# ehsan5890/optical-rl-gym-qot-aware

Hardware: AMD Instinct MI355X
Metric: env steps/sec (whole node) + blocking-prob parity, NSFNET RMSA 320 slots (higher is better)
Workload: dtype u64 bitmap + f64 statistics

## Files before the change

### optical-rl-gym-qot-aware_amd/csrc/orlg_api.hip

```cpp
#include "orlg_host.h"
#include "orlg_group_plan.h"
#include "orlg_wave.h"

struct orlg_env : OrlgHandle {
    OrlgParams p = {};
    int resident_blocks = 0;
    int group_mode = 0;
    OrlgGroupLayout group[3] = {};
    int group_usage_resident[ORLG_GROUP_WAVES + 1] = {};
    int group_resident[3][ORLG_GROUP_WAVES + 1] = {};
    uint4 *llog = nullptr;
    uint32_t *progress = nullptr;
    int allow_rejection = 0;
    std::vector<uint8_t> path_se;
    double *gn_table = nullptr;
    bool gn_protect = false;
    double *audit_table = nullptr;
};
enum { X_ACTIONS, X_GSNR, X_CAUSE, X_CAUSE_COUNTS, X_MARGIN };
static_assert(X_MARGIN < ORLG_EXTRA_SLOTS, "OrlgHandle::extra");

#define SYNC_CHECK(e) do { int rc_ = orlg_handle_sync_check(e); if (rc_) return rc_; } while (0)

__global__ void orlg_clear_state_kernel(OrlgParams p, int W, int keep_rng) {
    const size_t tid = (size_t)blockIdx.x * blockDim.x + threadIdx.x, nth = (size_t)gridDim.x * blockDim.x;
    for (size_t i = tid; i < (size_t)p.B * p.NW; i += nth) p.occ[i] = valid_mask(p.S, (int)(i % W));
    for (size_t i = tid; i < (size_t)p.B * p.Q; i += nth) {
        p.qtime[i] = __longlong_as_double((long long)ORLG_INF_BITS);
        p.qdesc[i] = 0;
    }
    for (size_t i = tid; i < (size_t)p.B * 4 * p.NBR; i += nth) p.hist[i] = 0;
    for (size_t i = tid; i < (size_t)p.B * 4 * p.E; i += nth) p.lstat[i] = 0.0;
    for (size_t i = tid; i < (size_t)p.B * p.lint_stride; i += nth) p.lint[i] = 0;
    for (size_t i = tid; i < (size_t)p.B; i += nth) {
        OrlgEnvScalars s;
        memset(&s, 0, sizeof(s));
        s.mt_idx = keep_rng ? p.scal[i].mt_idx : ORLG_MT_N;
        s.ring_pos = keep_rng ? p.scal[i].ring_pos : 0;
        s.ring_cnt = keep_rng ? p.scal[i].ring_cnt : 0;
        if (p.tr_arrival) { s.mt_idx = 0; s.ring_pos = 0; s.ring_cnt = 0; }
        p.scal[i] = s;
    }
}

__global__ __launch_bounds__(256) void orlg_simple_matrix_obs_kernel(const OrlgParams p, int W, uint8_t *out) {
    const size_t dim = (size_t)2 * p.N + (size_t)p.E * p.S;
    const size_t total = dim * p.B;
    for (size_t i = (size_t)blockIdx.x * blockDim.x + threadIdx.x; i < total; i += (size_t)gridDim.x * blockDim.x) {
        const size_t b = i / dim, q = i - b * dim;
        uint8_t v;
        if (q < (size_t)2 * p.N) {
            const OrlgEnvScalars *sc = p.scal + b;
            const int mn = sc->req_src < sc->req_dst ? sc->req_src : sc->req_dst;
            const int mx = sc->req_src < sc->req_dst ? sc->req_dst : sc->req_src;
            v = ((int)q == mn || (int)q == p.N + mx) ? 1 : 0;
        } else {
            const size_t r = q - 2 * p.N;
            const int link = (int)(r / p.S), s = (int)(r - (size_t)link * p.S);
            v = (uint8_t)((p.occ[b * p.NW + (size_t)link * W + (s >> 6)] >> (s & 63)) & 1ull);
        }
        out[i] = v;
    }
}

enum { EX_REQUEST, EX_COUNTERS, EX_TIME, EX_GRAPH, EX_RUNNING, EX_EPISODES, EX_HIST, EX_LSTAT };
__global__ void orlg_extract_kernel(OrlgParams p, int what, unsigned char *out) {
    const size_t tid = (size_t)blockIdx.x * blockDim.x + threadIdx.x, nth = (size_t)gridDim.x * blockDim.x;
    const size_t B = p.B;
    if (what == EX_REQUEST) {
        orlg_request *o = reinterpret_cast<orlg_request *>(out);
        for (size_t i = tid; i < B; i += nth) {
            const OrlgEnvScalars &s = p.scal[i];
            o[i].service_id = s.req_sid; o[i].src = s.req_src; o[i].dst = s.req_dst;
            o[i].bit_rate = reinterpret_cast<const int32_t *>(p.tables + p.t_bitrates)[s.req_br];
            o[i].arrival_time = s.req_arrival; o[i].holding_time = s.req_holding;
        }
    } else if (what == EX_COUNTERS) {
        int64_t *o = reinterpret_cast<int64_t *>(out);
        for (size_t i = tid; i < B * 8; i += nth) o[i] = p.scal[i / 8].c[i % 8];
    } else if (what == EX_TIME) {
        double *o = reinterpret_cast<double *>(out);
        for (size_t i = tid; i < B; i += nth) o[i] = p.scal[i].current_time;
    } else if (what == EX_GRAPH) {
        double *o = reinterpret_cast<double *>(out);
        for (size_t i = tid; i < B; i += nth) {
// ... 172 lines not shown


int orlg_create(const orlg_topology *t, const orlg_rmsa_config *c, int32_t batch, const uint64_t *seeds,
                uint64_t base_seed, int32_t device, orlg_env **out) {
    return orlg_create_traffic(t, c, batch, seeds, base_seed, device, nullptr, out);
}

static int rmsa_create(const orlg_topology *t, const orlg_rmsa_config *c, int32_t batch, const uint64_t *seeds, uint64_t base_seed,
                       int32_t device, const orlg_traffic *traffic, const orlg_trace *trace, orlg_env **out);
int orlg_create_traffic(const orlg_topology *t, const orlg_rmsa_config *c, int32_t batch, const uint64_t *seeds,
                        uint64_t base_seed, int32_t device, const orlg_traffic *traffic, orlg_env **out) {
    return rmsa_create(t, c, batch, seeds, base_seed, device, traffic, nullptr, out);
}
int orlg_create_trace(const orlg_topology *t, const orlg_rmsa_config *c, int32_t batch, int32_t device, const orlg_trace *trace,
                      orlg_env **out) {
    if (!trace) return fail(ORLG_ERR_INVALID, "null argument");
    return rmsa_create(t, c, batch, nullptr, 0, device, nullptr, trace, out);
}
int64_t orlg_trace_length(orlg_env *e) { return e ? e->trace.length : ORLG_ERR_INVALID; }
int64_t orlg_trace_position(orlg_env *e) { return e ? e->trace.position : ORLG_ERR_INVALID; }

static int rmsa_create(const orlg_topology *t, const orlg_rmsa_config *c, int32_t batch, const uint64_t *seeds, uint64_t base_seed,
                       int32_t device, const orlg_traffic *traffic, const orlg_trace *trace, orlg_env **out) {
    if (!t || !c || !out) return fail(ORLG_ERR_INVALID, "null argument");
    *out = nullptr;
    const int N = t->num_nodes, E = t->num_links, K = t->k_paths, S = c->num_slots, NBR = c->num_bit_rates;
    if (batch < 1) return fail(ORLG_ERR_INVALID, "batch must be >= 1");
    if (N < 2 || N > 64) return fail(ORLG_ERR_INVALID, "num_nodes %d not in 2..64", N);
    if (E < 1 || E > 255) return fail(ORLG_ERR_INVALID, "num_links %d not in 1..255", E);
    if (S < 1 || S > 512) return fail(ORLG_ERR_INVALID, "num_slots %d not in 1..512", S);
    const bool cont = c->bit_rate_cum == nullptr;
    if (NBR < 1 || NBR > (cont ? 256 : 64)) return fail(ORLG_ERR_INVALID, "num_bit_rates %d not in 1..%d", NBR, cont ? 256 : 64);
    if (cont) {
        if (!c->bit_rates) return fail(ORLG_ERR_INVALID, "null argument");
        for (int b = 1; b < NBR; b++)
            if (c->bit_rates[b] != c->bit_rates[0] + b) return fail(ORLG_ERR_INVALID, "continuous bit rates must be lower .. higher, one apart");
    }
    if (t->num_paths < 1 || t->num_paths >= (1 << 14)) return fail(ORLG_ERR_INVALID, "num_paths %d not in 1..16383", t->num_paths);
    int W = (S + 63) / 64;
    if (W == 7) W = 8;
    if (K < 1 || K * W > 64) return fail(ORLG_ERR_INVALID, "k_paths * words_per_link = %d exceeds one wavefront", K * W);
    if (c->j < 1 || c->j > 16) return fail(ORLG_ERR_INVALID, "j %d not in 1..16", c->j);
    if ((!traffic && !trace && (!(c->arrival_lambda > 0) || !(c->holding_lambda > 0))) || !(c->channel_width > 0))
        return fail(ORLG_ERR_INVALID, "arrival_lambda, holding_lambda and channel_width must be positive");
    auto e = std::make_unique<orlg_env>();
    double arrival_lambda = c->arrival_lambda, holding_lambda = c->holding_lambda;
    int rc = orlg_traffic_check(&e->traffic, traffic, batch, &arrival_lambda, &holding_lambda);
    if (rc) return rc;
    if (c->stats_level < 0 || c->stats_level > 2) return fail(ORLG_ERR_INVALID, "bad stats_level");
    for (int i = 0; i < N * N; i++) {
        int s = i / N, d = i % N;
        if (s != d && (t->pair_path_count[i] != K || t->pair_path_base[i] < 0 || t->pair_path_base[i] + K > t->num_paths))
            return fail(ORLG_ERR_INVALID, "pair (%d,%d) does not have k=%d path records", s, d, K);
    }
    const OrlgTraceState &trace_state = e->trace;
    if (trace) {
        if (!c->bit_rates) return fail(ORLG_ERR_INVALID, "null argument");
        rc = orlg_trace_check(&e->trace, &e->traffic, trace, batch, N, NBR, c->bit_rates, cont, &arrival_lambda, &holding_lambda);
        if (rc) return rc;
    }
    rc = orlg_handle_open(e.get(), device);
    if (rc) return rc;
    e->W = W; e->num_paths = t->num_paths;
    OrlgParams &p = e->p;
    p.err_flag = e->err.dev;
    p.B = batch; p.N = N; p.E = E; p.S = S; p.K = K; p.NBR = NBR; p.NW = E * W;
    p.episode_length = c->episode_length; p.reward_mode = c->reward_mode; p.stats_level = c->stats_level; p.j = c->j;
    p.obs_dim = 1 + 2 * N + (2 * c->j + 3) * K;
    p.arrival_lambda = arrival_lambda; p.holding_lambda = holding_lambda;
    int Q = c->queue_capacity;
    if (Q <= 0 && trace) {
        const int by_trace = trace_state.peak + 1, by_spectrum = E * S / 2 + 1;
        Q = by_trace < by_spectrum ? by_trace : by_spectrum;
        if (Q > 4096)
            return fail(ORLG_ERR_INVALID, "trace: up to %d services run at once (the trace's peak %d, the spectrum's bound %d): more than the 4096 "
                                          "release-queue slots the LDS holds", Q - 1, trace_state.peak, by_spectrum - 1);
    } else if (Q <= 0) {
        double load = arrival_lambda / holding_lambda;
        Q = (int)(load + 10.0 * std::sqrt(load));
    }
    Q = ((Q + 15) / 16) * 16;
    if (Q < 64) Q = 64;
    if (Q > 4096) return fail(ORLG_ERR_INVALID, "queue_capacity %d too large for LDS (max 4096)", Q);
    p.Q = Q;
    {
        char msg[192];
        snprintf(msg, sizeof(msg), "a release queue overflowed (capacity %d): the service stays provisioned and is never "
                                   "released -- raise queue_capacity", Q);
        e->overflow_message = msg;
    }

    auto up16 = [](int v) { return (v + 15) & ~15; };
    int off = 0;
    p.l_occ = off; off = up16(off + p.NW * 8);
    p.l_qtime = off; off = up16(off + Q * 8);
    p.l_qdesc = off; off = up16(off + Q * 4);
    p.l_mt = off; off = up16(off + ORLG_MT_N * 4);
    p.l_lstat = off; off = up16(off + 4 * E * 8);
    p.l_hist = off; off = up16(off + 4 * NBR * 4);
    p.lint_stride = (E + 3) & ~3;
    p.l_lint = off; off = up16(off + p.lint_stride * 4);
    p.l_scratch = off; off = up16(off + (int)sizeof(OrlgEnvScalars));
    p.l_wsc = off; off = up16(off + (int)sizeof(OrlgWaveScalars));
    p.l_ring = off; off = up16(off + ORLG_RING * (8 + 8 + 4));
    p.l_wave_bytes = off;

    {
        OrlgBlob blob;
        p.t_pair = blob.put(t->pair_path_base, (size_t)N * N * 4);
        std::vector<OrlgPathRec> recs;
        rc = orlg_path_records(t, E, "path %d: link %d out of range", &recs);
        if (rc) return rc;
        for (int g = 0; g < t->num_paths; g++)
            if (t->path_se[g] < 1 || t->path_se[g] >= ORLG_NSLOT_STRIDE)
                return fail(ORLG_ERR_INVALID, "path %d: spectral efficiency %d not in 1..7", g, t->path_se[g]);
        p.t_recs = blob.put(recs.data(), recs.size() * sizeof(OrlgPathRec));
        e->path_se.assign(t->path_se, t->path_se + t->num_paths);
        std::vector<uint16_t> ns((size_t)NBR * ORLG_NSLOT_STRIDE, 0);
        for (int b = 0; b < NBR; b++)
            for (int se = 1; se < ORLG_NSLOT_STRIDE; se++) {
                double q = (double)c->bit_rates[b] / ((double)se * c->channel_width);
                double n = std::ceil(q) + 1;
                ns[(size_t)b * ORLG_NSLOT_STRIDE + se] = (uint16_t)(n > 65535 ? 65535 : n);
            }
        p.t_nslots = blob.put(ns.data(), ns.size() * 2);
        p.t_bitrates = blob.put(c->bit_rates, (size_t)NBR * 4);
        {
            std::vector<double> zc((size_t)NBR, 0.0);
            p.t_brcum = blob.put(cont ? zc.data() : c->bit_rate_cum, (size_t)NBR * 8);
        }
        p.br_width = cont ? NBR : 0;
        p.t_srccum = blob.put(c->src_cum, (size_t)N * 8);
        p.t_dstcum = blob.put(c->dst_cum, (size_t)N * N * 8);
        if (c->stats_level >= ORLG_STATS_FULL) {
            std::vector<double> divs(S + 1), inv(S / 2 + 2);
            for (int k = 0; k <= S; k++) divs[k] = (double)k / (double)S;
            inv[0] = 0.0;
            for (size_t k = 1; k < inv.size(); k++) inv[k] = 1.0 / (double)k;
            p.t_divs = blob.put(divs.data(), divs.size() * 8);
            p.t_inv = blob.put(inv.data(), inv.size() * 8);
        }
        p.tab_bytes = (int32_t)blob.bytes.size();
        p.l_outs = p.tab_bytes;
        p.l_shared_bytes = p.tab_bytes + up16(ORLG_NUM_OUTS * 8);
        unsigned char *d_blob;
        rc = orlg_handle_upload(e.get(), &d_blob, blob.bytes.data(), blob.bytes.size());
        if (rc) return rc;
        p.tables = d_blob;
    }
    {
        const size_t lds_cu = ORLG_LDS_BYTES;
        int wpb = 0, best_waves = 0;
        const int wave_cap = 16;
        for (int cand = ORLG_MAX_WAVES_PER_BLOCK; cand >= 1; cand >>= 1) {
            size_t blk = (size_t)p.l_shared_bytes + (size_t)cand * p.l_wave_bytes;
            if (blk > lds_cu) continue;
            int waves = (int)(lds_cu / blk) * cand;
            if (waves > wave_cap) waves = wave_cap;
            if (waves > best_waves) { best_waves = waves; wpb = cand; }
        }
        if (wpb == 0) {
            size_t need = (size_t)p.l_shared_bytes + (size_t)p.l_wave_bytes;
            return fail(ORLG_ERR_INVALID, "tables + one environment (%zu B) exceed the 160 KiB LDS", need);
        }
        e->waves_per_block = wpb;
        e->lds_block_bytes = (size_t)p.l_shared_bytes + (size_t)wpb * p.l_wave_bytes;
// ... 943 lines not shown
```

### optical-rl-gym-qot-aware_amd/csrc/orlg_group_body.h

```cpp
    static_assert(!DEFER || (STATS >= 2 && !HBMQ), "the deferred link statistics belong to long launches with full statistics");
    static_assert(!(TRACE && TRAFFIC), "a trace handle has no arrival rates");
    static_assert(!LEAN || DEFER, "the lean body belongs to the long launches");
    static_assert(!CAUSE || (!HBMQ && !DEFER), "the blocking cause belongs to the plain kind");
    static_assert(!ASSIGN || (!HBMQ && !DEFER), "the assignment rules belong to the plain kind");
    static_assert(!CUT || ASSIGN, "the fewest-cuts window is an assignment rule");
    static_assert(!USAGE || (ASSIGN && !CUT), "most-used windows and the best-window route are assignment rules of their own");
    extern __shared__ __align__(16) unsigned char smem[];
    stage_tables(smem, p);
    const int lane = threadIdx.x & 63;
    const int wib = uni((int)(threadIdx.x >> 6));
    const int g = lane >> 4, gl = lane & 15;
    const Tab tb = make_tab(smem, p);
    uint32_t *mt_lds = reinterpret_cast<uint32_t *>(smem + p.l_shared_bytes);
    int *mt_lock = reinterpret_cast<int *>(smem + p.l_shared_bytes + p.g_mt);
    if (threadIdx.x == 0) *mt_lock = 0;
    __syncthreads();
    unsigned char *wbase = smem + p.l_shared_bytes + p.g_mt + 16 + (size_t)wib * p.g_wave_bytes;
    u64 *occ = reinterpret_cast<u64 *>(wbase + p.g_occ) + g * p.NW;
    double *qtime = nullptr;
    uint32_t *qdesc = nullptr;
    if constexpr (!HBMQ) {
        qtime = reinterpret_cast<double *>(wbase + p.g_qtime) + g * p.Q;
        qdesc = reinterpret_cast<uint32_t *>(wbase + p.g_qdesc) + g * p.Q;
    }
    double *lst = DEFER ? nullptr : reinterpret_cast<double *>(wbase + p.g_lstat) + g * 4 * p.E;
    int32_t *lint = reinterpret_cast<int32_t *>(wbase + p.g_lint) + g * p.lint_stride;
    u64 *lsum = DEFER ? reinterpret_cast<u64 *>(wbase + p.g_lstat) + g * p.E : nullptr;

    const int E = p.E, S = p.S, K = p.K, N = p.N, NBR = p.NBR, Q = p.Q, NW = p.NW;
    constexpr bool NET = STATS >= 1;
    constexpr bool FULL = STATS >= 2;
    const double INF = __longlong_as_double((long long)ORLG_INF_BITS);
    const bool out_comp = !LEAN && (p.out_mask & ((1 << ORLG_OUT_COMPACT) | (1 << ORLG_OUT_COMPACT_DIFF))) != 0;
    SEC_DECL_G

    const int n_quads = (p.B + ORLG_GE - 1) / ORLG_GE;
    const int n_chunks = p.n_chunks > 1 ? p.n_chunks : 1;
    const int n_tix = n_quads * n_chunks;
    const int n_waves = (int)(gridDim.x * (blockDim.x >> 6));
    const int n_static = n_chunks > 1 ? 0 : (n_waves < n_tix ? n_waves : n_tix);
    int tix = (int)(blockIdx.x * (blockDim.x >> 6)) + wib;
    if (n_chunks == 1 && tix >= n_tix) return;
    uint32_t nxt_tk = 0;
    if (n_chunks > 1 && lane == 0) nxt_tk = atomicAdd(p.ticket, 1u);
    for (bool first = n_chunks == 1;; first = false) {
    if (!first) {
        if (p.ticket_stride) {
            tix += n_waves;
            if (tix >= n_tix) break;
        } else {
            const uint32_t tk = (uint32_t)__builtin_amdgcn_readfirstlane((int)nxt_tk) - p.ticket_base;
            if (tk >= (uint32_t)(n_tix - n_static)) break;
            tix = n_static + (int)tk;
        }
    }
    int chunk = 0, quad = tix;
    if (n_chunks > 1) { chunk = tix / n_quads; quad = tix - chunk * n_quads; }
    const int t0 = n_chunks > 1 ? chunk * p.chunk_steps : 0;
    SEC(1);
    if (!p.ticket_stride && lane == 0) nxt_tk = atomicAdd(p.ticket, 1u);
    if (chunk > 0) {
        if (lane == 0)
            while (__hip_atomic_load(p.progress + quad, __ATOMIC_RELAXED, __HIP_MEMORY_SCOPE_AGENT) < (uint32_t)chunk) __builtin_amdgcn_s_sleep(16);
        __builtin_amdgcn_fence(__ATOMIC_ACQUIRE, "agent");
        asm volatile("s_waitcnt vmcnt(0)" ::: "memory");
    }
    const int env_raw = quad * ORLG_GE + g;
    const bool act = env_raw < p.B;
    const int env = act ? env_raw : p.B - 1;

    const int env0 = quad * ORLG_GE;
    const int nact = p.B - env0 < ORLG_GE ? p.B - env0 : ORLG_GE;
    quad_copy(wbase + p.g_occ, p.occ + (size_t)env0 * NW, nact * NW * 8, lane);
    if (FULL && !DEFER) quad_copy(wbase + p.g_lstat, p.lstat + (size_t)env0 * 4 * E, nact * 4 * E * 8, lane);
    int32_t *ghist = p.hist + (size_t)env * 4 * NBR;
    if (NET) quad_copy(wbase + p.g_lint, p.lint + (size_t)env0 * p.lint_stride, nact * p.lint_stride * 4, lane);
    if (nact < ORLG_GE) {
        wave_sync();
        if (!act) {
            const int gs_ = nact - 1;
            for (int i = gl; i < NW; i += ORLG_GL) occ[i] = (reinterpret_cast<u64 *>(wbase + p.g_occ) + gs_ * NW)[i];
            if (FULL && !DEFER) for (int i = gl; i < 4 * E; i += ORLG_GL) lst[i] = (reinterpret_cast<double *>(wbase + p.g_lstat) + gs_ * 4 * E)[i];
            if (NET) for (int i = gl; i < p.lint_stride; i += ORLG_GL) lint[i] = (reinterpret_cast<int32_t *>(wbase + p.g_lint) + gs_ * p.lint_stride)[i];
        }
    }
    uint4 *llog = DEFER ? p.llog + (size_t)env * E * ORLG_LLOG_CAP : nullptr;
    if (DEFER) lst = p.lstat + (size_t)env * 4 * E;
    bool need_replay = false;
    const OrlgEnvScalars *gs = p.scal + env;
    double current_time = gs->current_time, req_arrival = gs->req_arrival, req_holding = gs->req_holding;
    double g_thr = gs->g_throughput, g_comp = gs->g_compactness, g_lu = gs->g_last_update;
    long long cnt = gs->c[gl & 7];
    long long sum_bitrate_running = gs->sum_bitrate_running, episodes_done = gs->episodes_done;
    int sum_sh = gs->sum_slots_hops, n_running = gs->n_running;
    int req_src = gs->req_src, req_dst = gs->req_dst, req_br = gs->req_br, req_sid = gs->req_sid;
    int mt_idx = gs->mt_idx, new_service = gs->new_service, q_overflow = gs->q_overflow;
    int ring_pos = gs->ring_pos, ring_cnt = gs->ring_cnt;
    int sum_span = gs->sum_span, sum_gaps = gs->sum_gaps;
    int eproc = (int)gs->c[2];
    wave_sync();
    double comp_cur = 1.0;
    if (NET) comp_cur = network_compactness(sum_span, sum_sh, sum_gaps, E);
    if (DEFER)
        group_link_stats<W, true, false, true, 2>(lane, occ, nullptr, lint, tb, S, E, nullptr, E, 0.0, sum_span, sum_gaps, comp_cur,
                                                  0, 0.0, g_thr, g_comp, g_lu, nullptr, nullptr, lsum);
    int q_head = gs->q_head, q_n = n_running < Q ? n_running : Q;
    const int q_head0 = q_head;
    int q_pops = 0;
    if constexpr (HBMQ) {
        qtime = p.qtime + (size_t)env * Q;
        qdesc = p.qdesc + (size_t)env * Q;
    } else {
        const double *gqt = p.qtime + (size_t)env * Q;
        const uint32_t *gqd = p.qdesc + (size_t)env * Q;
        for (int j = gl; j < q_n; j += 2 * ORLG_GL) {
            int pos = q_head + j;
            pos -= pos >= Q ? Q : 0;
            int pos2 = pos + ORLG_GL;
            pos2 -= pos2 >= Q ? Q : 0;
            const bool two = j + ORLG_GL < q_n;
            const double t0 = gqt[pos];
            const uint32_t d0 = gqd[pos];
            double t1 = 0.0;
            uint32_t d1 = 0u;
            if (two) { t1 = gqt[pos2]; d1 = gqd[pos2]; }
            qtime[pos] = t0; qdesc[pos] = d0;
            if (two) { qtime[pos2] = t1; qdesc[pos2] = d1; }
        }
    }
    wave_sync();
    double next_rel = q_n > 0 ? qtime[q_head] : INF;
    uint32_t next_desc = q_n > 0 ? qdesc[q_head] : 0u;
    const int cidx = gl & 7;
    [[maybe_unused]] int cause_cnt = 0;
    int req_base = tb.pair_base[req_src * N + req_dst];

    const int n_iter = n_chunks > 1 ? (p.n_steps - t0 < p.chunk_steps ? p.n_steps - t0 : p.chunk_steps) : p.n_steps;
    const int policy = p.policy;
    for (int t = 0; t < n_iter; ++t) {
        SEC(2);
        double pf_iat = 0.0, pf_ht = 0.0;
        uint32_t pf_rq = 0;
        const bool pf_ok = ring_cnt > 0;
        if (pf_ok) {
            const size_t ro = (size_t)env * ORLG_RING + ring_pos;
            pf_iat = p.ring_iat[ro]; pf_ht = p.ring_ht[ro]; pf_rq = p.ring_req[ro];
        }
        const int base = req_base;
        int a_path = K, a_slot = S;
        int ff_n = 1, ff_hops = 0;
        if constexpr (ASSIGN) {
            constexpr int PP = ORLG_GL / W;
            const int rule = p.assign;
            const bool given = policy == ORLG_POLICY_PATH_EXT;
            int path0 = 0;
            bool a_ok = true;
            if (given) {
                const int a = p.actions[env];
                a_ok = a >= 0 && a < K;
                path0 = a_ok ? a : 0;
            }
            const bool llp = policy == ORLG_POLICY_LLP;
            const int kmax = (given || policy == ORLG_POLICY_SP) ? 1 : K;
            const int ps = gl / W, w = gl - ps * W;
            int found = 0x7fffffff, found_key = 0x7fffffff;
            [[maybe_unused]] const bool ranked = llp || policy == ORLG_POLICY_MIN_CUT;
            for (int p0 = 0; CUT && p0 < kmax; p0 += PP) {
                if (!ranked && ballot(act && a_ok && found == 0x7fffffff) == 0ull) break;
                const int pp = p0 + ps;
                const bool on = ps < PP && pp < kmax && a_ok;
                int hops_pp, n;
                u64 x;
                const uint32_t sk = seg_max<W>(cut_word_key<W>(occ, tb.recs, base + path0 + pp, w, on, tb.nslots + req_br * ORLG_NSLOT_STRIDE, S,
                                                               hops_pp, n, x));
                const bool head = on && w == 0 && sk != 0u;
                const int payload = head ? (((((path0 + pp) << 10) | cut_key_slot(sk)) << 14) | (n << 4) | hops_pp) : 0x7fffffff;
                if (ranked) {
                    const uint32_t fs = seg_add<W>((uint32_t)popc64(x));
                    const uint32_t rank = llp ? 1023u - fs : (uint32_t)cut_key_cuts(sk);
                    const int key = head ? (int)((rank << 6) | (uint32_t)pp) : 0x7fffffff;
                    const int bk = row_min_i32(key);
                    const int bp = row_min_i32(key == bk ? payload : 0x7fffffff);
                    if (bk < found_key) { found_key = bk; found = bp; }
                    continue;
                }
// ... 79 lines not shown
            const int ps = gl / W, w = gl - ps * W;
            int found = 0x7fffffff, found_key = 0x7fffffff;
            const u64 lastbit = (!deep && w == ((S - 1) >> 6)) ? 1ull << ((S - 1) & 63) : 0ull;
            for (int p0 = 0; p0 < kmax; p0 += PP) {
                if (!llp && ballot(act && a_ok && found == 0x7fffffff) == 0ull) break;
                const int pp = p0 + ps;
                const bool on = ps < PP && pp < kmax && a_ok;
                int se_pp, hops_pp;
                const u64 x = group_path_word_rec<W>(occ, tb.recs, base + path0 + pp, w, on, se_pp, hops_pp);
                int n = 1;
                if (on) n = tb.nslots[req_br * ORLG_NSLOT_STRIDE + se_pp];
                u64 r = run_starts<W>(x & ~lastbit, n, w);
                const u64 xprev = lane_prev_u64(x);
                if (deep) {
                    r &= x & ~((x << 1) | (w > 0 ? xprev >> 63 : 0ull));
                    if (!LEAN && policy == ORLG_POLICY_DEEP_EXT) {
                        const int cntw = popc64(r);
                        int incl = cntw, o;
                        o = lane_back_i32<1>(incl); incl += o;
                        o = lane_back_i32<2>(incl); incl += o;
                        o = lane_back_i32<4>(incl); incl += o;
                        const int kth = blk - (incl - cntw);
                        for (int q = 0; q < p.j; ++q)
                            if (q < kth) r &= r - 1;
                        if (kth < 0 || kth >= cntw) r = 0ull;
                    }
                }
                if (llp) {
                    const uint32_t fs = seg_add<W>((uint32_t)popc64(x));
                    const uint32_t fit = seg_max<W>(r ? (uint32_t)(0x7fff - (64 * w + ctz64(r))) : 0u);
                    const bool head = on && w == 0 && fit != 0u;
                    const int key = head ? (int)(((1023u - fs) << 6) | (uint32_t)pp) : 0x7fffffff;
                    const int bk = row_min_i32(key);
                    const int payload = (head && key == bk) ? ((((pp << 10) | (0x7fff - (int)fit)) << 14) | (n << 4) | hops_pp) : 0x7fffffff;
                    const int bp = row_min_i32(payload);
                    if (bk < found_key) { found_key = bk; found = bp; }
                    continue;
                }
                const int cand = r ? (((((path0 + pp) << 10) | (64 * w + ctz64(r))) << 14) | (n << 4) | hops_pp) : 0x7fffffff;
                const int best = row_min_i32(cand);
                if (found == 0x7fffffff) found = best;
            }
            if (found != 0x7fffffff) { a_path = found >> 24; a_slot = (found >> 14) & 1023; ff_n = (found >> 4) & 1023; ff_hops = found & 15; }
        }

        SEC(3);
        const double prev_compact = comp_cur;
        bool accepted = false;
        const bool in_range = act && a_path >= 0 && a_path < K && a_slot >= 0 && a_slot < S;
        const int gid = base + (in_range ? a_path : 0);
        const OrlgPathRec *rec = tb.recs + gid;
        int hops = ff_hops, n = ff_n;
        if (LEAN || policy != ORLG_POLICY_EXT) {
            accepted = in_range;
        } else {
            hops = rec->hops;
            n = tb.nslots[req_br * ORLG_NSLOT_STRIDE + rec->se];
            const bool on = in_range && gl < W;
            const u64 x = path_word<W>(occ, tb.recs, gid, gl < W ? gl : 0, on);
            const u64 m = on ? window_mask(a_slot, n, gl) : 0ull;
            const uint32_t bad = row_ballot((x & m) != m, lane);
            accepted = in_range && a_slot + n <= S && bad == 0u;
        }
        const int br_val = tb.bit_rates[req_br];
        [[maybe_unused]] int cause = 0;
        if constexpr (CAUSE) {
            const bool refused = act && !accepted;
            if (ballot(refused) != 0ull) {
                const int level = group_fit_level<W>(lane, occ, tb, base, K, S, req_br, refused);
                cause = refused ? ORLG_CAUSE_CAPACITY + level : ORLG_CAUSE_ACCEPTED;
            }
            if (act) cause_cnt += gl == cause ? 1 : 0;
        }
        if (!NET) group_apply_window<W>(lane, occ, rec->link, accepted ? hops : 0, a_slot, n, false);
        if (accepted) {
            sum_sh += n * hops;
            n_running += 1;
            sum_bitrate_running += br_val;
            cnt += (cidx == 1 || cidx == 3) ? 1 : ((cidx == 5 || cidx == 7) ? br_val : 0);
            if (gl == 0) { atomicAdd(ghist + NBR + req_br, 1); atomicAdd(ghist + 3 * NBR + req_br, 1); }
        }
        SEC(4);
        if (NET)
            group_link_stats<W, FULL, true, DEFER, DEFER ? 1 : 0, true>(lane, occ, lst, lint, tb, S, E, rec->link, accepted ? hops : 0,
                                                                          current_time, sum_span, sum_gaps, comp_cur, sum_sh,
                                                                          (double)sum_bitrate_running, g_thr, g_comp, g_lu, llog,
                                                                          &need_replay, lsum, a_slot, n);
        SEC(5);
        {
            const double rel = req_arrival + req_holding;
            bool ins = accepted && (act || !HBMQ);
            if (ins && q_n >= Q) { q_overflow = 1; ins = false; }
            bool down = false;
            if constexpr (!HBMQ) {
                if (ins && q_n > 0) {
                    int pm = q_head + (q_n >> 1);
                    pm -= pm >= Q ? Q : 0;
                    down = rel < qtime[pm];
                }
            }
            bool found = !ins || q_n == 0;
            int m = q_n;
            int left = q_n;
            int j = down ? gl : q_n - 1 - gl;
            int hd = down ? q_head - 1 : q_head + 1;
            hd = hd < 0 ? Q - 1 : (hd == Q ? 0 : hd);
            while (ballot(!found) != 0ull) {
                const bool scan = !found;
                const bool valid = scan && gl < left;
                int pos = q_head + j;
                pos -= pos >= Q ? Q : 0;
                double tq = 0.0;
                uint32_t dq = 0u;
                if (valid) { tq = qtime[pos]; dq = qdesc[pos]; }
                const bool moves = valid && (tq > rel) != down;
                int pos1 = hd + j;
                pos1 -= pos1 >= Q ? Q : 0;
                if (moves) { qtime[pos1] = tq; qdesc[pos1] = dq; }
                const uint32_t stay = row_ballot(valid && !moves, lane);
                if (scan) {
                    if (stay) { m = q_n - left + __builtin_ctz(stay); found = true; }
                    else if (left <= ORLG_GL) found = true;
                    else { left -= ORLG_GL; j += down ? ORLG_GL : -ORLG_GL; }
                }
            }
            if (ins) {
                const int r = down ? m : q_n - m;
                if (down) q_head = hd;
                int pr = q_head + r;
                pr -= pr >= Q ? Q : 0;
                const uint32_t desc = (uint32_t)gid | ((uint32_t)a_slot << 14) | ((uint32_t)req_br << 24);
                if (gl == 0) {
                    qtime[pr] = rel;
                    qdesc[pr] = desc;
                }
                q_n += 1;
                if (rel < next_rel) { next_rel = rel; next_desc = desc; }
            }
            wave_sync();
        }

        SEC(6);
        if (!LEAN && p.out_mask && act && gl == 0) {
            const size_t o = (size_t)(t0 + t) * p.B + env;
            const int om = p.out_mask;
            if (om & (1 << ORLG_OUT_PATH)) ORLG_GPTR(int32_t, tb.outs[ORLG_OUT_PATH])[o] = a_path;
            if (om & (1 << ORLG_OUT_SLOT)) ORLG_GPTR(int32_t, tb.outs[ORLG_OUT_SLOT])[o] = a_slot;
            if (om & (1 << ORLG_OUT_ACCEPTED)) ORLG_GPTR(uint8_t, tb.outs[ORLG_OUT_ACCEPTED])[o] = accepted ? 1 : 0;
            if (om & (1 << ORLG_OUT_REWARD))
                ORLG_GPTR(double, tb.outs[ORLG_OUT_REWARD])[o] =
                    p.reward_mode == 1 ? (accepted ? 1.0 : -1.0) : (accepted ? 1.0 : 0.0);
            if (om & (1 << ORLG_OUT_REQUEST))
                ORLG_GPTR(orlg_v4i, tb.outs[ORLG_OUT_REQUEST])[o] = orlg_v4i{req_sid, req_src, req_dst, br_val};
            if (om & (1 << ORLG_OUT_ARRIVAL)) ORLG_GPTR(double, tb.outs[ORLG_OUT_ARRIVAL])[o] = req_arrival;
            if (om & (1 << ORLG_OUT_HOLDING)) ORLG_GPTR(double, tb.outs[ORLG_OUT_HOLDING])[o] = req_holding;
            if (om & (1 << ORLG_OUT_COMPACT)) ORLG_GPTR(double, tb.outs[ORLG_OUT_COMPACT])[o] = comp_cur;
            if (om & (1 << ORLG_OUT_COMPACT_DIFF))
                ORLG_GPTR(double, tb.outs[ORLG_OUT_COMPACT_DIFF])[o] = prev_compact - comp_cur;
            if (FULL && (om & (1 << ORLG_OUT_AVG_LINK_COMPACT)))
                ORLG_GPTR(double, tb.outs[ORLG_OUT_AVG_LINK_COMPACT])[o] = np_mean(lst + 2 * E, E);
            if (FULL && (om & (1 << ORLG_OUT_AVG_LINK_UTIL)))
                ORLG_GPTR(double, tb.outs[ORLG_OUT_AVG_LINK_UTIL])[o] = np_mean(lst, E);
            if constexpr (CAUSE) {
                if (p.o_cause) ORLG_GPTR(uint8_t, p.o_cause)[o] = (uint8_t)cause;
            }
        }
        new_service = 0;

        SEC(7);
        {
// ... 99 lines not shown
                        const int pops = pair ? 2 : 1;
                        q_head += pops;
                        q_head -= q_head >= Q ? Q : 0;
                        q_pops += pops;
                        q_n -= pops;
                        n_running -= pops;
                        sum_bitrate_running -= br_a + (pair ? br_b : 0);
                        sum_sh -= n_a * hops_a + (pair ? n_b * hops_b : 0);
                        released = true;
                        next_rel = q_n > 0 ? qtime[q_head] : INF;
                        next_desc = q_n > 0 ? qdesc[q_head] : 0u;
                    }
                    const uint8_t *links2 = a_up ? (tb.recs + (int)(d_a & 0x3fff))->link : rec2->link;
                    group_release_links<W>(lane, occ, lsum, lint, S, links2, pair ? hop : gl, a_up ? hops_a : hops2,
                                           a_up ? (int)((d_a >> 14) & 0x3ff) : s0, a_up ? n_a : n2, current_time, sum_span, sum_gaps, llog,
                                           need_replay);
                    SEC(11);
                } else {
                    const uint32_t d = rel_now ? next_desc : 0u;
                    const int gid2 = (int)(d & 0x3fff), s0 = (int)((d >> 14) & 0x3ff), bri2 = (int)(d >> 24);
                    const OrlgPathRec *rec2 = tb.recs + gid2;
                    const int hops2 = rec2->hops;
                    const int n2 = tb.nslots[bri2 * ORLG_NSLOT_STRIDE + rec2->se];
                    if (rel_now) {
                        if (HBMQ && gl == 0) { qtime[q_head] = INF; qdesc[q_head] = 0u; }
                        q_head = q_head + 1 == Q ? 0 : q_head + 1;
                        q_pops += 1;
                        q_n -= 1;
                        n_running -= 1;
                        sum_bitrate_running -= tb.bit_rates[bri2];
                        sum_sh -= n2 * hops2;
                        released = true;
                    }
                    group_apply_window<W>(lane, occ, rec2->link, rel_now ? hops2 : 0, s0, n2, true);
                    if (rel_now) {
                        next_rel = q_n > 0 ? qtime[q_head] : INF;
                        next_desc = q_n > 0 ? qdesc[q_head] : 0u;
                    }
                    SEC(11);
                    if (NET)
                        group_link_stats<W, FULL, false, DEFER>(lane, occ, lst, lint, tb, S, E, rec2->link, rel_now ? hops2 : 0,
                                                                current_time, sum_span, sum_gaps, comp_cur, sum_sh, 0.0, g_thr, g_comp,
                                                                g_lu, llog, &need_replay);
                }
                if (DEFER && ballot(need_replay) != 0ull) {
                    SEC(14);
                    group_link_replay(lane, lst, lint, tb, S, E, llog);
                    need_replay = false;
                    SEC(11);
                }
            }
            if (NET && out_comp && released) comp_cur = network_compactness(sum_span, sum_sh, sum_gaps, E);
        }

        if (DEFER && ballot(need_replay) != 0ull) {
            SEC(14);
            group_link_replay(lane, lst, lint, tb, S, E, llog);
            need_replay = false;
        }
        SEC(12);
        {
            const bool done = act && eproc == p.episode_length;
            if (!LEAN && act && gl == 0 && (p.out_mask & (1 << ORLG_OUT_DONE)))
                ORLG_GPTR(uint8_t, tb.outs[ORLG_OUT_DONE])[(size_t)(t0 + t) * p.B + env] = done ? 1 : 0;
            if (ballot(done && p.auto_reset)) {
                if (done && p.auto_reset) {
                    for (int i = gl; i < NBR; i += ORLG_GL) { atomicExch(ghist + 2 * NBR + i, 0); atomicExch(ghist + 3 * NBR + i, 0); }
                    eproc = 1;
                    episodes_done += 1;
                    const int bv = tb.bit_rates[req_br];
                    if (cidx == 2) cnt = 1;
                    if (cidx == 3 || cidx == 7) cnt = 0;
                    if (cidx == 6) cnt = bv;
                }
                wave_sync();
                if (done && p.auto_reset && gl == 0) atomicExch(ghist + 2 * NBR + req_br, 1);
                wave_sync();
            }
        }
    }

    SEC(14);
    if (DEFER) group_link_replay(lane, lst, lint, tb, S, E, llog);
    SEC(13);
    wave_sync();
    {
        const int env0 = quad * ORLG_GE;
        const int nact = p.B - env0 < ORLG_GE ? p.B - env0 : ORLG_GE;
        quad_copy(p.occ + (size_t)env0 * NW, wbase + p.g_occ, nact * NW * 8, lane);
        if (FULL && !DEFER) quad_copy(p.lstat + (size_t)env0 * 4 * E, wbase + p.g_lstat, nact * 4 * E * 8, lane);
        if (NET) quad_copy(p.lint + (size_t)env0 * p.lint_stride, wbase + p.g_lint, nact * p.lint_stride * 4, lane);
    }
    if constexpr (CAUSE) {
        if (act && gl < ORLG_NUM_CAUSES && cause_cnt && p.o_cause_counts) atomicAdd(p.o_cause_counts + (size_t)env * ORLG_NUM_CAUSES + gl, cause_cnt);
    }
    if (act) {
        int q_headc = q_head;
        if constexpr (!HBMQ) {
            double *gqt = p.qtime + (size_t)env * Q;
            uint32_t *gqd = p.qdesc + (size_t)env * Q;
            q_headc = q_head0 + (int)((uint32_t)q_pops % (uint32_t)Q);
            q_headc -= q_headc >= Q ? Q : 0;
            int span = q_pops + q_n;
            span = span > Q ? Q : span;
            for (int j = gl; j < span; j += ORLG_GL) {
                int pos = q_head0 + j;
                pos -= pos >= Q ? Q : 0;
                int i = pos - q_headc;
                i += i < 0 ? Q : 0;
                int src = q_head + i;
                src -= src >= Q ? Q : 0;
                double tq = INF;
                uint32_t dq = 0u;
                if (i < q_n) { tq = qtime[src]; dq = qdesc[src]; }
                gqt[pos] = tq; gqd[pos] = dq;
            }
        }
        OrlgEnvScalars *go = p.scal + env;
        if (gl < 8) go->c[gl] = cnt;
        if (gl == 8) {
            go->current_time = current_time;
            go->req_arrival = req_arrival; go->req_holding = req_holding;
            go->g_throughput = g_thr; go->g_compactness = g_comp; go->g_last_update = g_lu;
            go->sum_bitrate_running = sum_bitrate_running;
            go->episodes_done = episodes_done;
            go->sum_slots_hops = sum_sh; go->n_running = n_running;
            go->req_src = req_src; go->req_dst = req_dst; go->req_br = req_br; go->req_sid = req_sid;
            go->mt_idx = mt_idx; go->new_service = new_service; go->q_overflow = q_overflow;
            go->ring_pos = ring_pos; go->ring_cnt = ring_cnt;
            go->sum_span = sum_span; go->sum_gaps = sum_gaps; go->q_head = q_headc;
            if (q_overflow) *p.err_flag = 1;
        }
    }
    wave_sync();
    if (n_chunks > 1) {
        asm volatile("s_waitcnt vmcnt(0)" ::: "memory");
        __builtin_amdgcn_fence(__ATOMIC_RELEASE, "agent");
        asm volatile("s_waitcnt vmcnt(0)" ::: "memory");
        if (lane == 0) __hip_atomic_store(p.progress + quad, (uint32_t)(chunk + 1), __ATOMIC_RELAXED, __HIP_MEMORY_SCOPE_AGENT);
    }
    SEC(0);
    }
    SEC_FLUSH;
```

### optical-rl-gym-qot-aware_amd/csrc/orlg_group_kernels.hip

```cpp
#pragma once
#include "orlg_link_stats.h"
#include "orlg_requests.h"
#include "orlg_sections.h"
#include "orlg_block_cause.h"
#include "orlg_assign.h"
#include "orlg_cut.h"
#include "orlg_usage.h"

#define ORLG_GL 16
#define ORLG_GE 4

DEV int row_add_i32(int v) { v += dpp_xor1(v); v += dpp_xor2(v); v += dpp_half_mirror(v); v += dpp_row_mirror(v); return v; }
DEV int row_swap8_i32(int v) { return __builtin_amdgcn_update_dpp(0, v, 0x128, 0xf, 0xf, false); }
DEV u64 half_row_or_u64(u64 v) {
    uint32_t lo = (uint32_t)v, hi = (uint32_t)(v >> 32);
    lo |= (uint32_t)dpp_xor1((int)lo); hi |= (uint32_t)dpp_xor1((int)hi);
    lo |= (uint32_t)dpp_xor2((int)lo); hi |= (uint32_t)dpp_xor2((int)hi);
    lo |= (uint32_t)dpp_half_mirror((int)lo); hi |= (uint32_t)dpp_half_mirror((int)hi);
    return ((u64)hi << 32) | lo;
}
DEV int row_min_i32(int v) {
    int o = dpp_xor1(v); v = o < v ? o : v;
    o = dpp_xor2(v); v = o < v ? o : v;
    o = dpp_half_mirror(v); v = o < v ? o : v;
    o = dpp_row_mirror(v); return o < v ? o : v;
}
DEV uint32_t row_ballot(bool p, int lane) { return (uint32_t)(ballot(p) >> (lane & 48)) & 0xffffu; }

#define ORLG_SEG_REDUCE(name, OP)                                                                   \
    template <int W>                                                                                \
    DEV uint32_t name(uint32_t v) {                                                                 \
        static_assert(W >= 1 && W <= 8 && W != 7, "words per link");                                \
        if (W == 1) return v;                                                                       \
        uint32_t o = (uint32_t)lane_ahead_i32<1>((int)v);                                           \
        const uint32_t s = OP(v, o);                                              \
        if (W == 2) return s;                                                                       \
        o = (uint32_t)lane_ahead_i32<2>((int)(W == 3 ? v : s));                                     \
        const uint32_t t = OP(s, o);                                      \
        if (W <= 4) return t;                                                                       \
        o = (uint32_t)lane_ahead_i32<4>((int)(W == 5 ? v : (W == 6 ? s : t)));                      \
        return OP(t, o);                                                      \
    }
#define ORLG_OP_ADD(a, b) ((a) + (b))
#define ORLG_OP_MAX(a, b) ((a) > (b) ? (a) : (b))
ORLG_SEG_REDUCE(seg_add, ORLG_OP_ADD)
ORLG_SEG_REDUCE(seg_max, ORLG_OP_MAX)
#undef ORLG_SEG_REDUCE

template <int W>
DEV u64 group_path_word_rec(const u64 *occ, const OrlgPathRec *recs, int gid, int w, bool active, int &se, int &hops_out) {
    uint4 r = make_uint4(0u, 0u, 0u, 0u);
    if (active) r = *reinterpret_cast<const uint4 *>(recs + gid);
    const uint32_t q[4] = {r.x, r.y, r.z, r.w};
    const int hops = (int)(r.x & 0xffu);
    se = (int)((r.x >> 8) & 0xffu);
    hops_out = hops;
    u64 acc = active ? ~0ull : 0ull;
#pragma unroll
    for (int h0 = 0; h0 < ORLG_MAX_HOPS; h0 += 4) {
        if (ballot(h0 < hops) == 0ull) break;
        u64 v[4] = {~0ull, ~0ull, ~0ull, ~0ull};
#pragma unroll
        for (int k = 0; k < 4; ++k) {
            const int h = h0 + k;
            if (h < ORLG_MAX_HOPS) {
                const int link = (int)((q[(h + 2) >> 2] >> (8 * ((h + 2) & 3))) & 0xffu);
                v[k] = occ[__mul24(link, W) + w];
            }
        }
#pragma unroll
        for (int k = 0; k < 4; ++k) acc &= v[k];
    }
    return acc;
}

DEV u64 lsum_pack(int freec, int F, int U, int lmin, int lmax, int ml, bool ff, bool lf) {
    return (u64)((uint32_t)freec | ((uint32_t)F << 10) | ((uint32_t)U << 20)) |
           ((u64)((uint32_t)(lmin & 0x3ff) | ((uint32_t)lmax << 10) | ((uint32_t)ml << 20) | ((uint32_t)ff << 30) | ((uint32_t)lf << 31)) << 32);
}

template <int W, bool LINKF, bool GRAPH, bool DEFER = false, int SUM = 0, bool APPLY = false>
DEV void group_link_stats(const int lane, u64 *occ, double *lst, int32_t *lint, const Tab &tb, int S, int E, const uint8_t *links,
                          int nlinks, double now, int &sum_span, int &sum_gaps, double &comp_cur, int sum_sh, double cur_thr,
                          double &g_thr, double &g_comp, double &g_lu, uint4 *llog = nullptr, bool *need_replay = nullptr,
                          u64 *lsum = nullptr, int win_s = 0, int win_n = 0) {
    static_assert(W <= 8, "at least two links per row");
    static_assert(!APPLY || SUM != 2, "the summary rebuild changes no occupancy");
    static_assert(SUM == 0 || (LINKF && DEFER && (SUM == 1 || !GRAPH)), "summaries belong to the deferred instantiation");
    constexpr int NS = ORLG_GL / W;
    const int gl = lane & 15;
// ... 115 lines not shown

template <int W>
DEV void group_release_links(const int lane, u64 *occ, u64 *lsum, int32_t *lint, int S, const uint8_t *links, int hop, int hops, int s,
                             int n, double now, int &sum_span, int &sum_gaps, uint4 *llog, bool &need_replay) {
    static_assert(ORLG_MAX_HOPS <= ORLG_GL, "one lane per hop");
    int dspan = 0, dgaps = 0;
    if (hop < hops) {
        const int link = (int)links[hop];
        u64 *lw = occ + __mul24(link, W);
        const int e = s + n;
        const int ia = s > 0 ? (s - 1) >> 6 : 0, ib = e < S ? e >> 6 : 0, ws = s >> 6, we = (e - 1) >> 6;
        const u64 xa = lw[ia], xb = lw[ib], xs = lw[ws], xe = lw[we];
        const u64 sm = lsum[link];
        const u64 hm = ~0ull << (s & 63), lm = ~0ull >> (63 - ((e - 1) & 63));
        if (ws == we) {
            lw[ws] = xs | (hm & lm);
        } else {
            lw[ws] = xs | hm;
            for (int j = ws + 1; j < we; ++j) lw[j] = ~0ull;
            lw[we] = xe | lm;
        }
        int p = -1, q = 64 * W;
        if (s > 0) {
            const u64 y = ~xa & (~0ull >> (63 - ((s - 1) & 63)));
            if (y) p = 64 * ia + 63 - clz64(y);
            else
                for (int j = ia - 1; j >= 0; --j) {
                    const u64 v = ~lw[j];
                    if (v) { p = 64 * j + 63 - clz64(v); break; }
                }
        }
        if (e < S) {
            const u64 y = ~xb & (~0ull << (e & 63));
            if (y) q = 64 * ib + ctz64(y);
            else
                for (int j = ib + 1; j < W; ++j) {
                    const u64 v = ~lw[j];
                    if (v) { q = 64 * j + ctz64(v); break; }
                }
        } else {
            q = e;
        }
        const int L = s - 1 - p, R = q - e;
        const uint32_t lo32 = (uint32_t)sm, hi32 = (uint32_t)(sm >> 32);
        const int freec = (int)(lo32 & 0x3ff) + n;
        const int F = (int)((lo32 >> 10) & 0x3ff) + 1 - (L > 0) - (R > 0);
        const int U = (int)((lo32 >> 20) & 0x3ff) + (s > 0 && L == 0) + (e < S && R == 0) - 1;
        int lmin = (int)(hi32 & 0x3ff);
        int lmax = (int)((hi32 >> 10) & 0x3ff);
        int ml = (int)((hi32 >> 20) & 0x3ff);
        const bool ff = ((hi32 >> 30) & 1u) || s == 0, lf = (hi32 >> 31) || e == S;
        ml = L + n + R > ml ? L + n + R : ml;
        if (U == 0) { lmin = 0x7fff; lmax = 0; }
        else {
            if (lmin == s) lmin = e + R;
            if (lmax == e) lmax = s - L;
        }
        lsum[link] = lsum_pack(freec, F, U, lmin, lmax, ml, ff, lf);
        const int nspan = U > 1 ? lmax - lmin : 0, ngaps = U > 1 ? U - 1 : 0;
        int old = lint[link];
        int cnt = (int)((uint32_t)old >> 26);
        const int max_empty = (F > 1 && !(F == 2 && ff && lf)) ? ml : 0;
        if (cnt < ORLG_LLOG_CAP - 1) {
            llog[__mul24(link, ORLG_LLOG_CAP) + cnt] =
                make_uint4((uint32_t)freec | ((uint32_t)max_empty << 10) | ((uint32_t)(lmax - lmin) << 20), (uint32_t)U,
                           (uint32_t)__double2loint(now), (uint32_t)__double2hiint(now));
            cnt += 1;
        }
        if (cnt >= ORLG_LLOG_FLUSH) need_replay = true;
        old &= 0x03ffffff;
        lint[link] = nspan | (ngaps << 16) | (cnt << 26);
        dspan = nspan - (old & 0xffff);
        dgaps = ngaps - (old >> 16);
    }
    sum_span += row_add_i32(dspan);
    sum_gaps += row_add_i32(dgaps);
    wave_sync();
}

DEV void group_link_replay(const int lane, double *lst, int32_t *lint, const Tab &tb, int S, int E, const uint4 *llog) {
    link_replay<ORLG_GL>(lane, lst, lint, tb, S, E, llog);
}

template <int W>
DEV void group_apply_window(int lane, u64 *occ, const uint8_t *links, int hops, int s, int n, bool set_free) {
    constexpr int HPP = ORLG_GL / W;
    const int gl = lane & 15;
    const int hs = gl / W, w = gl - hs * W;
    const u64 m = window_mask(s, n, w);
    for (int h0 = 0;; h0 += HPP) {
        if (ballot(h0 < hops) == 0ull) break;
        const int h = h0 + hs;
        if (hs < HPP && h < hops && m) {
            u64 *word = occ + __mul24((int)links[h], W) + w;
            *word = set_free ? (*word | m) : (*word & ~m);
        }
    }
    wave_sync();
}

DEV void quad_copy(void *dst, const void *src, int bytes, int lane) {
    const int n16 = bytes >> 4;
    const uint4 *s16 = reinterpret_cast<const uint4 *>(src);
    uint4 *d16 = reinterpret_cast<uint4 *>(dst);
    for (int i0 = 0; i0 < n16; i0 += 4 * ORLG_WAVE) {
        uint4 v[4];
#pragma unroll
        for (int k = 0; k < 4; ++k) {
            const int i = i0 + k * ORLG_WAVE + lane;
            v[k] = make_uint4(0u, 0u, 0u, 0u);
            if (i < n16) v[k] = s16[i];
        }
#pragma unroll
        for (int k = 0; k < 4; ++k) {
            const int i = i0 + k * ORLG_WAVE + lane;
            if (i < n16) d16[i] = v[k];
        }
    }
    if ((bytes & 8) && lane == 0) reinterpret_cast<u64 *>(dst)[2 * n16] = reinterpret_cast<const u64 *>(src)[2 * n16];
}

template <int W>
DEV int group_fit_level(int lane, const u64 *occ, const Tab &tb, int base, int K, int S, int br, bool need) {
    constexpr int PP = ORLG_GL / W;
    const int gl = lane & 15;
    const int ps = gl / W, w = gl - ps * W;
    int top = 0;
    for (int p0 = 0; p0 < K; p0 += PP) {
        const int pp = p0 + ps;
        const bool on = need && ps < PP && pp < K;
        int se_pp, hops_pp;
        const u64 x = group_path_word_rec<W>(occ, tb.recs, base + pp, w, on, se_pp, hops_pp);
        int n = 1;
        if (on) n = tb.nslots[br * ORLG_NSLOT_STRIDE + se_pp];
        const int lv = on ? window_level(run_starts<W>(x, n, w), n, S, w) : 0;
        const int row = row_ballot(lv == 4, lane) ? 4 : (row_ballot(lv == 3, lane) ? 3 : 0);
        top = row > top ? row : top;
    }
    const bool more = need && top < 3;
    if (ballot(more) == 0ull) return top;
    for (int idp = 0; idp < K; ++idp) {
        if (ballot(more && top < 2) == 0ull) break;
        const OrlgPathRec *rec = tb.recs + (base + idp);
        const int hops = more && top < 2 ? (int)rec->hops : 0;
        const int n = tb.nslots[br * ORLG_NSLOT_STRIDE + rec->se];
        uint32_t nocap = 0u, norun = 0u;
        for (int h0 = 0;; h0 += PP) {
            if (ballot(h0 < hops) == 0ull) break;
            const int h = h0 + ps;
            const bool on = ps < PP && h < hops;
            u64 x = 0ull;
            if (on) x = occ[__mul24((int)rec->link[on ? h : 0], W) + w];
            const uint32_t freec = seg_add<W>((uint32_t)popc64(x));
            const uint32_t has = seg_max<W>(run_starts<W>(x, n, w) != 0ull ? 1u : 0u);
            const bool head = on && w == 0;
            nocap |= row_ballot(head && (int)freec < n, lane);
            norun |= row_ballot(head && has == 0u, lane);
        }
        const int lv = nocap ? 0 : (norun ? 1 : 2);
        if (more && lv > top) top = lv;
    }
    return top;
}

template <int W, int STATS, bool HBMQ, bool DEFER, bool TRAFFIC, bool TRACE, bool LEAN>
DEV void orlg_rmsa_group_body(const OrlgParams &p) {
// ... 19 lines not shown
```

Before: 1.671 billion.

## Defer lean-body graph throughput/compactness updates into a packed per-lane replay log

```diff
diff --git a/optical-rl-gym-qot-aware_amd/csrc/orlg_api.hip b/optical-rl-gym-qot-aware_amd/csrc/orlg_api.hip
--- a/optical-rl-gym-qot-aware_amd/csrc/orlg_api.hip
+++ b/optical-rl-gym-qot-aware_amd/csrc/orlg_api.hip
@@ -1,6 +1,7 @@
 #include "orlg_host.h"
 #include "orlg_group_plan.h"
 #include "orlg_wave.h"
+#include "orlg_graph_log.h"
 
 struct orlg_env : OrlgHandle {
     OrlgParams p = {};
@@ -339,6 +340,7 @@
     Q = ((Q + 15) / 16) * 16;
     if (Q < 64) Q = 64;
     if (Q > 4096) return fail(ORLG_ERR_INVALID, "queue_capacity %d too large for LDS (max 4096)", Q);
+    static_assert(4096 <= ORLG_GLOG_MAX_Q, "the lean body's graph log packs the bit rates of a full queue (orlg_graph_log.h)");
     p.Q = Q;
     {
         char msg[192];
diff --git a/optical-rl-gym-qot-aware_amd/csrc/orlg_graph_log.h b/optical-rl-gym-qot-aware_amd/csrc/orlg_graph_log.h
--- /dev/null
+++ b/optical-rl-gym-qot-aware_amd/csrc/orlg_graph_log.h
@@ -0,0 +1,64 @@
+#pragma once
+#if defined(__HIPCC__)
+#include "orlg_wave.h"
+#endif
+#include "orlg_math.h"
+
+#define ORLG_GLOG_FN ORLG_HD __attribute__((always_inline))
+#define ORLG_GLOG_CAP 16
+#define ORLG_GLOG_MAX_ES (255 * 512)
+#define ORLG_GLOG_MAX_Q 4096
+#define ORLG_GLOG_SUM_BITS 17
+#define ORLG_GLOG_BR_BITS 45
+static_assert(ORLG_GLOG_MAX_ES < (1 << ORLG_GLOG_SUM_BITS), "an E S sum must fit its field");
+static_assert((long long)ORLG_GLOG_MAX_Q * 0x7fffffffLL < (1LL << ORLG_GLOG_BR_BITS), "the bit rates of a full queue must fit their field");
+static_assert(3 * ORLG_GLOG_SUM_BITS + ORLG_GLOG_BR_BITS == 96, "three registers");
+
+struct OrlgGraphEntry {
+    double now;
+    uint32_t w0, w1, w2;
+};
+
+ORLG_GLOG_FN void orlg_glog_pack(OrlgGraphEntry &e, double now, long long sum_bitrate_running, int sum_span, int sum_sh, int sum_gaps) {
+    const uint64_t br = (uint64_t)sum_bitrate_running;
+    e.now = now;
+    e.w0 = (uint32_t)sum_span | ((uint32_t)sum_sh << 17);
+    e.w1 = ((uint32_t)sum_sh >> 15) | ((uint32_t)sum_gaps << 2) | ((uint32_t)(br >> 32) << 19);
+    e.w2 = (uint32_t)br;
+}
+
+struct OrlgGraphTerm {
+    double now, ynow;
+    double c_thr, c_comp;
+};
+
+ORLG_GLOG_FN OrlgGraphTerm orlg_glog_eval(const OrlgGraphEntry &e, double prev, int E) {
+    const int sum_span = (int)(e.w0 & 0x1ffffu), sum_sh = (int)((e.w0 >> 17) | ((e.w1 & 3u) << 15)), sum_gaps = (int)((e.w1 >> 2) & 0x1ffffu);
+    const long long br = (long long)(((uint64_t)(e.w1 >> 19) << 32) | e.w2);
+    OrlgGraphTerm t;
+    t.now = e.now;
+    t.ynow = 0.0;
+    t.c_thr = 0.0;
+    t.c_comp = 0.0;
+    double comp = 1.0;
+    if (sum_gaps > 0) comp = ORLG_FDIV((double)sum_span, (double)sum_sh) * ORLG_FDIV((double)E, (double)sum_gaps);
+    if (e.now > 0) {
+#if defined(__HIP_DEVICE_COMPILE__)
+        t.ynow = recip_refine(e.now);
+#endif
+        const double time_diff = e.now - prev;
+        t.c_thr = (double)br * time_diff;
+        t.c_comp = comp * time_diff;
+    }
+    return t;
+}
+
+ORLG_GLOG_FN double orlg_glog_chain(double g, double g_lu, double c, double now, double ynow) {
+    const double num = (g * g_lu) + c;
+#if defined(__HIP_DEVICE_COMPILE__)
+    return div_by(num, now, ynow);
+#else
+    (void)ynow;
+    return num / now;
+#endif
+}
diff --git a/optical-rl-gym-qot-aware_amd/csrc/orlg_group_body.h b/optical-rl-gym-qot-aware_amd/csrc/orlg_group_body.h
--- a/optical-rl-gym-qot-aware_amd/csrc/orlg_group_body.h
+++ b/optical-rl-gym-qot-aware_amd/csrc/orlg_group_body.h
@@ -99,8 +99,10 @@
     int sum_span = gs->sum_span, sum_gaps = gs->sum_gaps;
     int eproc = (int)gs->c[2];
     wave_sync();
+    [[maybe_unused]] OrlgGraphEntry lg = {0.0, 0u, 0u, 0u};
+    [[maybe_unused]] int lg_cnt = 0;
     double comp_cur = 1.0;
-    if (NET) comp_cur = network_compactness(sum_span, sum_sh, sum_gaps, E);
+    if (NET && !LEAN) comp_cur = network_compactness(sum_span, sum_sh, sum_gaps, E);
     if (DEFER)
         group_link_stats<W, true, false, true, 2>(lane, occ, nullptr, lint, tb, S, E, nullptr, E, 0.0, sum_span, sum_gaps, comp_cur,
                                                   0, 0.0, g_thr, g_comp, g_lu, nullptr, nullptr, lsum);
@@ -346,10 +348,21 @@
         }
         SEC(4);
         if (NET)
-            group_link_stats<W, FULL, true, DEFER, DEFER ? 1 : 0, true>(lane, occ, lst, lint, tb, S, E, rec->link, accepted ? hops : 0,
-                                                                          current_time, sum_span, sum_gaps, comp_cur, sum_sh,
-                                                                          (double)sum_bitrate_running, g_thr, g_comp, g_lu, llog,
-                                                                          &need_replay, lsum, a_slot, n);
+            group_link_stats<W, FULL, !LEAN, DEFER, DEFER ? 1 : 0, true>(lane, occ, lst, lint, tb, S, E, rec->link, accepted ? hops : 0,
+                                                                           current_time, sum_span, sum_gaps, comp_cur, sum_sh,
+                                                                           (double)sum_bitrate_running, g_thr, g_comp, g_lu, llog,
+                                                                           &need_replay, lsum, a_slot, n);
+        if constexpr (LEAN) {
+            const bool logs = accepted && hops > 0;
+            OrlgGraphEntry ne;
+            orlg_glog_pack(ne, current_time, sum_bitrate_running, sum_span, sum_sh, sum_gaps);
+            if (logs && gl == lg_cnt) lg = ne;
+            lg_cnt += logs ? 1 : 0;
+            if (ballot(lg_cnt >= ORLG_GLOG_CAP) != 0ull) {
+                SEC(15);
+                group_graph_replay(lane, lg, lg_cnt, p.scal + env, E);
+            }
+        }
         SEC(5);
         {
             const double rel = req_arrival + req_holding;
@@ -615,6 +628,10 @@
 
     SEC(14);
     if (DEFER) group_link_replay(lane, lst, lint, tb, S, E, llog);
+    if constexpr (LEAN) {
+        SEC(15);
+        if (ballot(lg_cnt > 0) != 0ull) group_graph_replay(lane, lg, lg_cnt, p.scal + env, E);
+    }
     SEC(13);
     wave_sync();
     {
@@ -654,7 +671,7 @@
         if (gl == 8) {
             go->current_time = current_time;
             go->req_arrival = req_arrival; go->req_holding = req_holding;
-            go->g_throughput = g_thr; go->g_compactness = g_comp; go->g_last_update = g_lu;
+            if (!LEAN) { go->g_throughput = g_thr; go->g_compactness = g_comp; go->g_last_update = g_lu; }
             go->sum_bitrate_running = sum_bitrate_running;
             go->episodes_done = episodes_done;
             go->sum_slots_hops = sum_sh; go->n_running = n_running;
diff --git a/optical-rl-gym-qot-aware_amd/csrc/orlg_group_kernels.hip b/optical-rl-gym-qot-aware_amd/csrc/orlg_group_kernels.hip
--- a/optical-rl-gym-qot-aware_amd/csrc/orlg_group_kernels.hip
+++ b/optical-rl-gym-qot-aware_amd/csrc/orlg_group_kernels.hip
@@ -6,6 +6,7 @@
 #include "orlg_assign.h"
 #include "orlg_cut.h"
 #include "orlg_usage.h"
+#include "orlg_graph_log.h"
 
 #define ORLG_GL 16
 #define ORLG_GE 4
@@ -287,6 +288,36 @@
     link_replay<ORLG_GL>(lane, lst, lint, tb, S, E, llog);
 }
 
+static_assert(255 * 64 * ORLG_MAX_W <= ORLG_GLOG_MAX_ES, "a link is a byte, a link's bitmap ORLG_MAX_W words: the log's E S fields");
+DEV void group_graph_replay(const int lane, const OrlgGraphEntry &lg, int &cnt, OrlgEnvScalars *gs, int E) {
+    const int gl = lane & 15;
+    __builtin_amdgcn_fence(__ATOMIC_RELEASE, "workgroup");
+    __builtin_amdgcn_fence(__ATOMIC_ACQUIRE, "workgroup");
+    const bool head = gl == 0 && cnt > 0;
+    double x_thr = 0.0, x_comp = 0.0, g_lu = 0.0;
+    if (head) { x_thr = gs->g_throughput; x_comp = gs->g_compactness; g_lu = gs->g_last_update; }
+    const double before = ORLG_DPP_F64(lane_prev_i32, lg.now);
+    const double lu = gl == 0 ? g_lu : before;
+    const OrlgGraphTerm t = orlg_glog_eval(lg, lu, E);
+    const bool upd = gl < cnt && t.now > 0;
+    const int c0 = __builtin_amdgcn_readlane(cnt, 0), c1 = __builtin_amdgcn_readlane(cnt, 16);
+    const int c2 = __builtin_amdgcn_readlane(cnt, 32), c3 = __builtin_amdgcn_readlane(cnt, 48);
+    const int m01 = c0 > c1 ? c0 : c1, m23 = c2 > c3 ? c2 : c3;
+    const int nmax = m01 > m23 ? m01 : m23;
+    double o_thr = 0.0, o_comp = 0.0;
+    for (int k = 0; k < nmax; ++k) {
+        const double n_thr = orlg_glog_chain(x_thr, lu, t.c_thr, t.now, t.ynow);
+        const double n_comp = orlg_glog_chain(x_comp, lu, t.c_comp, t.now, t.ynow);
+        o_thr = upd ? n_thr : x_thr;
+        o_comp = upd ? n_comp : x_comp;
+        x_thr = ORLG_DPP_F64(lane_prev_i32, o_thr);
+        x_comp = ORLG_DPP_F64(lane_prev_i32, o_comp);
+    }
+    if (gl == nmax - 1 && cnt > 0) { gs->g_throughput = o_thr; gs->g_compactness = o_comp; }
+    if (gl == cnt - 1) gs->g_last_update = lg.now;
+    cnt = 0;
+}
+
 template <int W>
 DEV void group_apply_window(int lane, u64 *occ, const uint8_t *links, int hops, int s, int n, bool set_free) {
     constexpr int HPP = ORLG_GL / W;
```

Result: faster. 1.704 billion, median of 6 (+2.0%).
